# hidasib/GRU4Rec

Hardware: NVIDIA H100
Metric: mini-batches/sec (higher is better)
Workload: dtype f32

## Files before the change

### gru4rec_b200/csrc/g4r_fast.cuh

```cuda
#pragma once

constexpr int FK_THREADS = 512;
constexpr int FK_NW = FK_THREADS / 32;
constexpr int FK_G = 48;
constexpr int FK_CT = 32;
constexpr int FK_Q = FK_CT / FK_NW;
constexpr int FK_B = 32;
static_assert(FK_THREADS / 16 == FK_B, "statistics mapping: 16 threads per lane");
constexpr int FK_LDS = 132;


__device__ __forceinline__ void red_release_add(unsigned int* p, unsigned int v) {
  asm volatile("red.release.gpu.global.add.u32 [%0], %1;" :: "l"(p), "r"(v) : "memory");
}
__device__ __forceinline__ unsigned int atom_acqrel_add(unsigned int* p, unsigned int v) {
  unsigned int old;
  asm volatile("atom.acq_rel.gpu.global.add.u32 %0, [%1], %2;" : "=r"(old) : "l"(p), "r"(v) : "memory");
  return old;
}
__device__ __forceinline__ void wait_ge(const unsigned int* p, unsigned int target) {
  while (ld_acquire_u32(p) < target) { }
}
__device__ __forceinline__ uint32_t smem_u32(const void* p) { return (uint32_t)__cvta_generic_to_shared(p); }
__device__ __forceinline__ void mbar_init(uint64_t* bar, unsigned int count) {
  asm volatile("mbarrier.init.shared::cta.b64 [%0], %1;" :: "r"(smem_u32(bar)), "r"(count) : "memory");
}
__device__ __forceinline__ void mbar_expect_tx(uint64_t* bar, unsigned int bytes) {
  asm volatile("mbarrier.arrive.expect_tx.shared::cta.b64 _, [%0], %1;" :: "r"(smem_u32(bar)), "r"(bytes) : "memory");
}
__device__ __forceinline__ void mbar_wait(uint64_t* bar, unsigned int parity) {
  asm volatile(
      "{\n\t.reg .pred p;\n\t"
      "WAIT_LOOP:\n\t"
      "mbarrier.try_wait.parity.shared::cta.b64 p, [%0], %1;\n\t"
      "@p bra.uni WAIT_DONE;\n\t"
      "bra.uni WAIT_LOOP;\n\t"
      "WAIT_DONE:\n\t}\n" :: "r"(smem_u32(bar)), "r"(parity) : "memory");
}
__device__ __forceinline__ void tma_row(void* sdst, const void* gsrc, unsigned int bytes, uint64_t* bar) {
  asm volatile("cp.async.bulk.shared::cluster.global.mbarrier::complete_tx::bytes [%0], [%1], %2, [%3];"
               :: "r"(smem_u32(sdst)), "l"(gsrc), "r"(bytes), "r"(smem_u32(bar)) : "memory");
}

struct FastSmem {
  alignas(128) float sY[FK_B * FK_LDS];
  float sS[FK_CT * FK_LDS];
  float sAcc[FK_CT * FK_LDS];
  float sVel[FK_CT * FK_LDS];
  float sTW[FK_B * FK_LDS];
  float sD[FK_CT * FK_LDS];
  float sG[FK_CT * FK_B];
  float sO[FK_CT * FK_B];
  float sRS[FK_B * 8];
  float sPart[FK_NW * FK_B * 8];
// ... 597 lines not shown
    while (je < nj && sm.sIt[buf][je] == item) je++;
    if (lane < kw) {
      const float4 p0 = ld4(sm.sS + j * FK_LDS + lane * 4), z = make_float4(0.f, 0.f, 0.f, 0.f);
      RowChain<float4> u;
      u.begin(p0, p0, ada ? ld4(sm.sAcc + j * FK_LDS + lane * 4) : z, mom ? ld4(sm.sVel + j * FK_LDS + lane * 4) : z);
      for (int k = j; k < je; k++) u.add(md, ld4(sm.sD + k * FK_LDS + lane * 4), ada, mom);
      const size_t off = (size_t)item * ldL + lane * 4;
      st4(md.Wy + off, u.ps);
      if (ada) st4(md.Wy_acc + off, u.al);
      if (mom) st4(md.Wy_vel + off, u.vl);
    }
    if (lane == 0) {
      RowChain<float> u;
      u.begin(sm.sByP[j], sm.sByP[j], sm.sByA[j], sm.sByV[j]);
      for (int k = j; k < je; k++) u.add(md, sm.sDby[k], ada, mom);
      md.By[item] = u.ps;
      if (ada) md.By_acc[item] = u.al;
      if (mom) md.By_vel[item] = u.vl;
    }
  }
}
template <class SM>
__device__ __forceinline__ void fk_dby(SM& sm, int M, int nj) {
  const int lane = threadIdx.x & 31, warp = threadIdx.x >> 5;
  for (int jj = warp; jj < nj; jj += FK_NW) {
    float a = (lane < M) ? sm.sG[jj * FK_B + lane] : 0.f;
    a = warp_sum(a);
    if (lane == 0) sm.sDby[jj] = a;
  }
}
#include "g4r_fastc.cuh"

template <bool CL>
__global__ void __launch_bounds__(FK_THREADS, 1) k_fast_t(int slot, int n_steps, FastSync* fs, unsigned long long* tstamp) {
  using SM = typename std::conditional<CL, FastSmemC, FastSmemR>::type;
  extern __shared__ __align__(128) unsigned char fk_raw[];
  SM& sm = *reinterpret_cast<SM*>(fk_raw);
  const ModelDev& md = MD;
  const LayerDev& ly = md.layer[0];
  const int cta = blockIdx.x, ncta = gridDim.x;
  const int tid = threadIdx.x, lane = tid & 31, warp = tid >> 5;
  const int G = CL ? (int)cl_size() : md.ldL / 4;
  const bool gru = cta < G;
  const bool col = CL || !gru;
  const int chunk = CL ? cta : cta - G;
  const int ncol = CL ? ncta : ncta - G;
  const bool has_chunk = col && chunk < md.NCH;
  const bool pw = loss_pairwise(md.loss);
  const int ldL = md.ldL, B = md.B;
  const int kw = ldL / 4;
  uint64_t* bar = reinterpret_cast<uint64_t*>(&sm.mbar);
  unsigned int bar_epoch = 0, gepoch = 0, stats_target = 0;
  const int in_ctas = min(B, ncta - G);
#ifdef G4R_CF_FINE
#define FK_FTS(s_) ((tstamp && cta == 0 && (s_) < 500 && n_steps >= 1000) ? tstamp + (size_t)((s_) + 500) * 16 : nullptr)
#define FK_STAMP_OK(s_) ((s_) < 500)
#else
#define FK_FTS(s_) ((unsigned long long*)nullptr)
#define FK_STAMP_OK(s_) true
#endif
#define FK_STAMP(k) do { if (tstamp && cta == ((CL || ((k) >= 4 && (k) <= 8)) ? 0 : G) && tid == 0 && FK_STAMP_OK(s)) { unsigned long long t_; asm volatile("mov.u64 %0, %%globaltimer;" : "=l"(t_)); tstamp[(size_t)s * 16 + (k)] = t_; } } while (0)
  if (tid == 0) { mbar_init(bar, 1); asm volatile("fence.mbarrier_init.release.cluster;" ::: "memory"); }
  if (col) fk_load_idx(md, sm, 0, n_steps, chunk, 0);
  __syncthreads();
  if (col) fk_prefetch_rows(md, sm, 0, n_steps, 0, pw);
  ClusterCtx cc = {0, 1, 0, 0};
  if constexpr (CL) {
    if (gru) {
      cc = cf_init(md, sm);
      cf_load_resident(md, sm, cc);
      if (n_steps > 0) {
        fk_stage_lanes(md, sm, 0, md.wM[0]);
        cf_f1(md, sm, cc, 0, false, nullptr, 0u, nullptr);
        cf_f2(md, sm, cc, 0, nullptr);
        __syncthreads();
        if (tid == 0) red_release_add(&fs->h_ready, 1u);
      }
    }
  } else {
    if (gru) {
      fr_load_resident(md, sm, 4 * cta);
      if (n_steps > 0) {
        fk_stage_lanes(md, sm, 0, md.wM[0]);
        stage_rows4(sm.gH[0], FK_LDS, FK_B, kw, [&](int rr) -> const float* { const int sl = sm.gIdx[rr]; return sl >= 0 ? ly.H + (size_t)sl * ldL : nullptr; });
        fr_f1(md, sm, 0, 4 * cta, sm.gH[0], nullptr, 0u);
// ... 142 lines not shown
      const int b = chunk;
      const bool maxed = !(md.loss == G4R_LOSS_BPR || md.loss == G4R_LOSS_TOP1);
      float mc = -INFINITY, Z = 0.f, A = 0.f, Q = 0.f, D = 0.f, T = 0.f, has = 0.f, tt = 0.f;
      if (tid < md.NCH) {
        const float* st = md.stat + ((size_t)tid * md.B + b) * G4R_NSTAT;
        const float4 u = ld4(st), v = ld4(st + 4);
        mc = u.x; Z = u.y; A = u.z; Q = u.w; D = v.x; T = v.y; has = v.z;
        if (tid == 0) tt = v.w;
      }
      float mg = mc;
#pragma unroll
      for (int o = 1; o < 32; o <<= 1) mg = fmaxf(mg, __shfl_xor_sync(0xffffffffu, mg, o));
      if (lane == 0) sm.sPart[warp] = mg;
      __syncthreads();
      mg = sm.sPart[0];
      for (int w = 1; w < FK_NW; w++) mg = fmaxf(mg, sm.sPart[w]);
      if (loss_softmaxneg(md.loss)) mg = fmaxf(mg, 0.f);
      if (maxed) {
        const float sc = (mc == -INFINITY) ? 0.f : expf(mc - mg);
        Z *= sc; A *= sc; Q *= sc; D *= sc;
      }
#pragma unroll
      for (int o = 1; o < 32; o <<= 1) {
        Z += __shfl_xor_sync(0xffffffffu, Z, o); A += __shfl_xor_sync(0xffffffffu, A, o); Q += __shfl_xor_sync(0xffffffffu, Q, o);
        D += __shfl_xor_sync(0xffffffffu, D, o); T += __shfl_xor_sync(0xffffffffu, T, o); has += __shfl_xor_sync(0xffffffffu, has, o);
      }
      __syncthreads();
      if (lane == 0) { float* w = sm.sPart + 32 + warp * 8; w[0] = Z; w[1] = A; w[2] = Q; w[3] = D; w[4] = T; w[5] = has; w[6] = tt; }
      __syncthreads();
      if (tid == 0) {
        tt = sm.sPart[32 + 6];
        for (int w = 1; w < FK_NW; w++) { const float* q = sm.sPart + 32 + w * 8; Z += q[0]; A += q[1]; Q += q[2]; D += q[3]; T += q[4]; }
        const float m = mg;
        float* rs = md.RS + (size_t)b * G4R_NSTAT;
        float loss = 0.f, r0 = m, r1 = Z, r2 = 0.f, r3 = 0.f, r4 = 0.f, r5 = tt;
        if (md.loss == G4R_LOSS_XE) { const float pt = __fdiv_rn(expf(T - m), Z); loss = -logf(pt + G4R_EPS_LOG); r2 = pt; r5 = T; }
        else if (md.loss == G4R_LOSS_XE_LOGIT) { loss = logf(Z) - (T - m); r5 = T; }
        else if (md.loss == G4R_LOSS_BPR_MAX) { r2 = __fdiv_rn(A, Z); r3 = __fdiv_rn(Q, Z); r4 = __fdiv_rn(D, Z); loss = -logf(r2 + G4R_EPS_LOG) + md.bpreg * r3; }
        else if (md.loss == G4R_LOSS_TOP1_MAX) { r2 = __fdiv_rn(A, Z); r4 = __fdiv_rn(D, Z); loss = r2; }
        else if (md.loss == G4R_LOSS_BPR) { loss = A; r4 = D; }
        else { const float c = sigmoidf_(tt * tt); loss = (float)M * (__fdiv_rn(A, (float)N) - __fdiv_rn(c, (float)(M + md.S_cfg))); r4 = D; }
        st4(rs, make_float4(r0, r1, r2, r3));
        st4(rs + 4, make_float4(r4, r5, loss, 0.f));
        red_release_add(&fs->stats, 1u);
      }
    }
    stats_target += (unsigned int)M;
    if (tid == 0) wait_ge(&fs->stats, stats_target);
    __syncthreads();
    FK_STAMP(2);
    if (tid < M * 2) st4(sm.sRS + tid * 4, ld4(md.RS + tid * 4));
    __syncthreads();
    if (chunk == 0 && tid == 0) {
      float c = 0.f;
      for (int b = 0; b < M; b++) c += sm.sRS[b * 8 + 6];
      c = __fdiv_rn(c, (float)md.B);
      md.cost[s] = c;
      if (c != c) atomicExch(md.nanflag, 1);
    }
    FK_STAMP(11);
    for (int i = tid; i < FK_CT * FK_B; i += FK_THREADS) {
      const int jj = i / FK_B, b = i % FK_B;
      sm.sG[i] = (jj < nj && b < M) ? loss_grad_elem(md, sm.sRS + (size_t)b * 8, sm.sO[i], sm.sTc[buf][b] == cb + jj, M, N) : 0.f;
    }
    __syncthreads();
    fk_dby(sm, M, nj);
    FK_STAMP(12);
    float* part = md.part + (size_t)(has_chunk ? chunk : 0) * md.B * ldL;
    if constexpr (CL) {
      if (has_chunk) { fk_dsy(sm, M, nj, kw); fk_part(sm, part, M, nj, ldL); }
      __syncthreads();
      FK_STAMP(13);
      fk_update_rows(md, sm, buf, nj, kw);
      if (has_chunk && nj == 0) for (int i = tid; i < M * ldL; i += FK_THREADS) part[i] = 0.f;
      __syncthreads();
      FK_STAMP(14);
      bar_epoch += 1;
      if (tid == 0) { red_release_add(&fs->bar, 1u); wait_ge(&fs->bar, bar_epoch * (unsigned int)ncta); }
      __syncthreads();
      FK_STAMP(3);
      fk_b1<CL>(md, sm, s, cta, ncta);
      __syncthreads();
      if (tid == 0) red_release_add(&fs->b1_done, 1u);
      FK_STAMP(15);
      fk_prefetch_rows(md, sm, s + 1, n_steps, buf ^ 1, pw);
      FK_STAMP(4);
      if (gru) {
        if (s + 1 < n_steps) fk_stage_lanes(md, sm, s + 1, md.wM[s + 1]);
        cf_backward(md, sm, cc, fs, s, ncta, s + 1 < n_steps, (tstamp && cta == 0 && FK_STAMP_OK(s)) ? tstamp + (size_t)s * 16 : nullptr, FK_FTS(s));
        FK_STAMP(6);
        if (s + 1 < n_steps) {
          cf_f1(md, sm, cc, s + 1, true, &fs->in_done, (unsigned int)(s + 1) * (unsigned int)in_ctas, FK_FTS(s));
          FK_STAMP(7);
          cf_f2(md, sm, cc, s + 1, FK_FTS(s));
          __syncthreads();
          if (tid == 0) red_release_add(&fs->h_ready, 1u);
        } else {
          cl_wait();
        }
        FK_STAMP(8);
      }
      if (!gru && cta < G + in_ctas) {
        const unsigned int tgt = (unsigned int)(s + 1) * (unsigned int)G;
        if (in_ctas == B && ly.ld3 / 4 <= FK_THREADS) fk_sparse_in_one(md, sm, s, cta - G, &fs->grp, tgt);
        else {
          if (tid == 0) wait_ge(&fs->grp, tgt);
          __syncthreads();
          for (int b = cta - G; b < B; b += in_ctas) { fk_sparse_in(md, sm, s, b); __syncthreads(); }
        }
        __syncthreads();
        if (tid == 0) red_release_add(&fs->in_done, 1u);
      }
    } else {
      if (has_chunk) fk_part(sm, part, M, nj, ldL);
      if (has_chunk && nj == 0) for (int i = tid; i < M * ldL; i += FK_THREADS) part[i] = 0.f;
      __syncthreads();
      FK_STAMP(13);
      bar_epoch += 1;
      if (tid == 0) { red_release_add(&fs->bar, 1u); wait_ge(&fs->bar, bar_epoch * (unsigned int)ncol); }
      __syncthreads();
      FK_STAMP(3);
      fk_b1<CL>(md, sm, s, chunk, ncol);
      __syncthreads();
      if (tid == 0) red_release_add(&fs->b1_done, 1u);
      FK_STAMP(15);
      fk_dsy(sm, M, nj, kw);
      __syncthreads();
      if (chunk < in_ctas) {
        const unsigned int tgt = (unsigned int)(s + 1) * (unsigned int)G;
        if (in_ctas == B && ly.ld3 / 4 <= FK_THREADS) fk_sparse_in_one(md, sm, s, chunk, &fs->dvec_done, tgt);
        else {
          if (tid == 0) wait_ge(&fs->dvec_done, tgt);
          __syncthreads();
          for (int b = chunk; b < B; b += in_ctas) { fk_sparse_in(md, sm, s, b); __syncthreads(); }
        }
        __syncthreads();
        if (tid == 0) red_release_add(&fs->in_done, 1u);
      }
      fk_update_rows(md, sm, buf, nj, kw);
      __syncthreads();
      FK_STAMP(14);
      if (tid == 0) red_release_add(&fs->rows_done, 1u);
      if (s + 1 < n_steps) {
        if (tid == 0) wait_ge(&fs->rows_done, (unsigned int)(s + 1) * (unsigned int)ncol);
        __syncthreads();
        fk_prefetch_rows(md, sm, s + 1, n_steps, buf ^ 1, pw);
      }
    }
  }
  if constexpr (CL) { if (gru) cf_store_resident(md, sm, cc); }
  else { if (gru) fr_store_resident(md, sm, 4 * cta); }
#undef FK_STAMP
}
```

### gru4rec_b200/csrc/g4r_kernels.cuh

```cuda
#pragma once
#include <cuda_runtime.h>
#include <stdint.h>
#include "../../include/g4r.h"

#define G4R_EPS_LOG 1e-24f
#define G4R_NSTAT 8

struct ActSpec { int kind; float p1, p2; };
constexpr int MG_CAP = 256;
struct MgDev {
  int R, rank;
  int *gItem, *gPos, *gM, *gX;
  int *mEnt, *mItem, *mCbeg;
  int *mTot;
  int *xEnt, *xItem, *xTot;
  float *DSYall, *DBYall, *INall;
  float* gradFlat; size_t gradCount;
};

struct MgTensor { float *p, *acc, *vel; size_t goff; int count; };
struct TsBuf {
  unsigned char *A1, *A2, *A3, *A4, *A5, *A6, *A7, *A8;
  unsigned char *W1, *W2, *W3, *W4, *B3, *B4, *B5, *B8a, *B8b;
  float *P, *P1, *Pa, *Pb;
// ... 26 lines not shown

constexpr int MGS_MAXR = 8;
constexpr int MGS_FLAG_STRIDE = 32;
constexpr int MGS_GRU_CTAS = 48;
enum { MGF_ROWS = 0, MGF_APPLIED = MGS_MAXR, MGF_IN = 2 * MGS_MAXR, MGF_INAPPLIED = 3 * MGS_MAXR, MGF_DENSE = 4 * MGS_MAXR,
       MGF_COUNT = 4 * MGS_MAXR + MGS_MAXR * MGS_GRU_CTAS };
struct ShardDev {
  int R, rank, rows_local, ldW;
  int NA, DSL;
  float* W[MGS_MAXR];
  float* Wx[MGS_MAXR];
  float* inbox[MGS_MAXR];
  float* inboxIn[MGS_MAXR];
  float* denseIn[MGS_MAXR];
  float* mgInLL[MGS_MAXR];
  unsigned int* flags[MGS_MAXR];
  float *W_acc, *W_vel, *Wx_acc, *Wx_vel;
  float* mgIn;
  const int *aEnt, *aItem, *aCbeg;
  const int *xEnt, *xItem, *xTot;
  const int *gX, *gM;
  int* abort;
};
struct FastSync {
  unsigned int bar;      unsigned int p0[31];
  unsigned int stats;    unsigned int p1[31];
  unsigned int h_ready;  unsigned int p2[31];
  unsigned int b1_done;  unsigned int p3[31];
  unsigned int grp;      unsigned int p4[31];
  unsigned int in_done;  unsigned int p5[31];
  unsigned int dvec_done; unsigned int p6[31];
  unsigned int rows_done; unsigned int p7[31];
};
struct GridBar { unsigned int count; unsigned int gen; unsigned int pad[30]; };

struct LayerDev {
  int L, ldL, ld2, ld3;
  int in_dim, ld_in;
  float *Wx, *Wx_acc, *Wx_vel;
  float *Wh, *Wh_acc, *Wh_vel;
  float *Wrz, *Wrz_acc, *Wrz_vel;
  float *Bh, *Bh_acc, *Bh_vel;
  float *Wx_g, *Wh_g, *Wrz_g, *Bh_g;
  float *H;
  float *Hold, *r, *z, *ah, *ht, *y;
  float *dvec;
  float *dy;
  float *Hr;
  const float* in;
};

struct ModelDev {
  int n_items, n_layers, B, Bld, S, mode;
  int L, ldL;
  int in0_dim, ld_in0;
  int NP;
  int NCH;
  int loss; ActSpec fact, hact;
  float p_drop_h, p_drop_e, lr, mom, lmbd, bpreg, logq, alpha;
  int adapt; int nn_top1;
  float ap1, ap1c, ap2, ap2c;
  float grad_cap, smoothing;
  const float* gscale;
  float* gnorm2;
  float* stat2;
  int S_cfg;
// ... 1125 lines not shown
```

### gru4rec_b200/csrc/g4r_lib.cu

```cuda
#include <cuda_runtime.h>
#include <cub/device/device_radix_sort.cuh>
#include <algorithm>
#include <cmath>
#include <cstdio>
#include <cstring>
#include <map>
#include <mutex>
#include <string>
#include <vector>
#include "g4r_kernels.cuh"
#include "g4r_misc.cuh"

#define G4R_VERSION 102

static thread_local std::string g_create_error;
struct g4r_handle;
static void eval_release(g4r_handle* h);
static void sessions_release(g4r_handle* h);
static void mg_release(g4r_handle* h);
static void shard_release(g4r_handle* h);
static bool shard_eligible(const g4r_config& c, int n_sm);
static int shard_create(g4r_handle* h);
static bool tc_eligible(const g4r_config& c);
struct TensorInfo;
// ... 63 lines not shown
  std::string err;
  cudaStream_t stream = nullptr;
  cudaEvent_t ev0 = nullptr, ev1 = nullptr;
  char* ws = nullptr; size_t ws_bytes = 0; bool own_ws = false;
  size_t ws_off = 0;
  std::map<std::string, TensorInfo> tensors;
  int Bmax = 0, n_sm = 132;
  int CAP = 0;
  int *hX = nullptr, *hY = nullptr, *hSlot = nullptr, *hM = nullptr, *hSti = nullptr; uint8_t* hF = nullptr; uint32_t* hG = nullptr;
  float* hCost = nullptr;
  int *dX = nullptr, *dY = nullptr, *dSlot = nullptr, *dM = nullptr, *dSti = nullptr, *dXnext = nullptr; uint8_t *dF = nullptr, *dXflag = nullptr; uint32_t* dG = nullptr;
  int* dStepBase = nullptr;
  float *dP = nullptr, *dLogP0t = nullptr, *dLogP0s = nullptr, *dU = nullptr;
  int* dST = nullptr; int gen_len = 0; int64_t sample_ptr = 0; bool have_store = false; bool have_cdf = false;
  int32_t* dMrgState = nullptr; int n_streams = 0; bool mrg_init = false; int64_t mrg_rstate[6];
  float* He[G4R_MAX_LAYERS] = {};
  int* dRankCnt = nullptr; float* dTgt = nullptr;
  uint32_t global_step = 0;
  int win_steps = 0;
  int64_t launches = 0;
  int npow2 = 0;
  int slot = -1;
  cudaGraphExec_t graphU = nullptr, graph1 = nullptr; int graph_unroll = 16;
  bool use_graph = true;
  GridBar* dGridBar = nullptr; unsigned long long* dStamp = nullptr; int pk_blocks = 0; size_t pk_smem = 0;
  bool mg_alloc = false; MgDev mgdev; std::vector<MgTensor> mg_tensors;
  void* eval_ctx = nullptr;
  void* sessions = nullptr;
  uint64_t wy_version = 0;
  void* mg_host = nullptr;
  void* shard = nullptr;
  char* shard_ws = nullptr;
  size_t shard_ws_bytes = 0;
  FastSync* dFastSync = nullptr; bool fast_ok = false; bool fastc_ok = false; int fastc_grid = 0; int* hFlags = nullptr; int64_t fast_windows = 0, slow_windows = 0;
  bool prof = false; bool stamp_on = false;
  bool two_pass = false;
  bool phase_only = false;
  float* dGscale = nullptr;
  bool tc_ok = false; void* ts_buf = nullptr; unsigned long long* ts_dbg = nullptr; cudaStream_t side = nullptr, side2 = nullptr; cudaEvent_t ts_ev[12] = {};
  std::vector<cudaEvent_t> prof_ev; std::vector<int> prof_phase;
  BpttDev bw = {}; void* bptt_cub = nullptr; size_t bptt_cub_bytes = 0; int64_t bptt_windows = 0;
  FullDev fs = {}; int64_t full_steps = 0;
};

enum { PH_GATHER = 0, PH_F1, PH_F2, PH_SCORE, PH_STATS, PH_LOSSGRAD, PH_B1, PH_B2, PH_B3, PH_DENSE, PH_SPARSE_IN, PH_STATS2, PH_GRADCAP, PH_COUNT };
static const char* kPhaseNames[PH_COUNT] = {"gather_in", "gru_rz", "gru_h", "score", "stats", "lossgrad_update", "gru_bwd_elem", "gru_bwd_dHr", "gru_bwd_din", "dense_update", "sparse_in_update",
                                            "smoothing_stats", "grad_cap_norm_apply"};

#define LAUNCH_ON(strm, ph, ...) do { \
    cudaEvent_t e0_ = nullptr, e1_ = nullptr; \
    if (h->prof) { cudaEventCreate(&e0_); cudaEventCreate(&e1_); cudaEventRecord(e0_, (strm)); } \
    __VA_ARGS__; \
    h->launches++; \
    if (h->prof) { cudaEventRecord(e1_, (strm)); h->prof_ev.push_back(e0_); h->prof_ev.push_back(e1_); h->prof_phase.push_back(ph); } \
  } while (0)
#define LAUNCH(ph, ...) LAUNCH_ON(h->stream, ph, __VA_ARGS__)

#define CK(call) do { cudaError_t e_ = (call); if (e_ != cudaSuccess) { h->err = std::string(#call) + ": " + cudaGetErrorString(e_); return G4R_ERR_CUDA; } } while (0)
#define FAIL(code, msg) do { h->err = (msg); return (code); } while (0)

static inline int round4(int x) { return (x + 3) & ~3; }
static inline size_t align_up(size_t x, size_t a) { return (x + a - 1) / a * a; }

struct Carver {
  char* base; size_t off; bool dry;
  template <class T> T* take(size_t n) {
// ... 104 lines not shown
    ly.Hold = cv.take<float>((size_t)Bmax * ly.ldL); ly.r = cv.take<float>((size_t)Bmax * ly.ldL); ly.z = cv.take<float>((size_t)Bmax * ly.ldL);
    ly.ah = cv.take<float>((size_t)Bmax * ly.ldL); ly.ht = cv.take<float>((size_t)Bmax * ly.ldL); ly.y = cv.take<float>((size_t)Bmax * ly.ldL);
    ly.dvec = cv.take<float>((size_t)Bmax * ly.ld3); ly.dy = cv.take<float>((size_t)Bmax * ly.ldL); ly.Hr = cv.take<float>((size_t)Bmax * ly.ldL);
    reg("y" + si, ly.y, Bmax, L, ly.ldL); reg("dvec" + si, ly.dvec, Bmax, 3 * L, ly.ld3);
  }
  if (mode != 0) {
    md.Sx = cv.take<float>((size_t)Bmax * md.ld_in0); md.in0 = cv.take<float>((size_t)Bmax * md.ld_in0); md.dSx = cv.take<float>((size_t)Bmax * md.ld_in0);
    if (mode == 2) { md.snapAcc = cv.take<float>((size_t)Bmax * md.ld_in0); md.snapVel = cv.take<float>((size_t)Bmax * md.ld_in0); }
    reg("dSx", md.dSx, Bmax, md.in0_dim, md.ld_in0);
  }
  for (int i = 0; i < nl; i++) md.layer[i].in = (i == 0) ? md.in0 : md.layer[i - 1].y;
  md.O = cv.take<float>((size_t)NP * md.Bld);
  md.DSY = cv.take<float>((size_t)NP * ldL); md.DBY = cv.take<float>((size_t)NP);
  const FullDev fsh = full ? full_shape(c, n_sm) : FullDev{};
  md.part = cv.take<float>((size_t)std::max(NCH, fsh.ks) * B * ldL);
  md.stat = cv.take<float>((size_t)NCH * B * G4R_NSTAT);
  md.RS = cv.take<float>((size_t)Bmax * G4R_NSTAT);
  md.stat2 = md.smoothing > 0.f ? cv.take<float>((size_t)NCH * B * 2) : nullptr;
  float* gsc = c.grad_cap > 0.f ? cv.take<float>(8) : nullptr;
  md.gscale = gsc;
  md.cost = cv.take<float>((size_t)CAP);
  md.nanflag = cv.take<int>(4);
  reg("O", md.O, NP, Bmax, md.Bld); reg("DSY", md.DSY, NP, Llast, ldL);
  int* dX = cv.take<int>((size_t)CAP * B); int* dY = cv.take<int>((size_t)CAP * B); int* dSlot = cv.take<int>((size_t)CAP * B);
  int* dXnext = cv.take<int>((size_t)CAP * B);
  uint8_t* dF = cv.take<uint8_t>((size_t)CAP * B); uint8_t* dXflag = cv.take<uint8_t>((size_t)CAP * B);
  int* dM = cv.take<int>(CAP); int* dSti = cv.take<int>(CAP); uint32_t* dG = cv.take<uint32_t>(CAP);
  md.pItem = cv.take<int>((size_t)CAP * NP); md.pPos = cv.take<int>((size_t)CAP * NP);
  md.pTcol = cv.take<int>((size_t)CAP * B); md.pCbeg = cv.take<int>((size_t)CAP * (NCH + 1));
  md.pKey = shard ? cv.take<int>((size_t)CAP * NP) : nullptr;
  int* dStepBase = cv.take<int>(4);
  GridBar* dGridBar = cv.take<GridBar>(1);
  FastSync* dFastSync = cv.take<FastSync>(1);
  unsigned long long* dStamp = cv.take<unsigned long long>((size_t)CAP * 16);
  float* dP = cv.take<float>(c.n_items); float* dL0t = cv.take<float>(c.n_items); float* dL0s = cv.take<float>(c.n_items);
  int* dST = store ? cv.take<int>((size_t)gen_len * c.n_sample) : nullptr;
  float* dU = store ? cv.take<float>((size_t)gen_len * c.n_sample) : nullptr;
  int32_t* dMrg = cv.take<int32_t>((size_t)15360 * 6);
  MgDev mgd; memset(&mgd, 0, sizeof(mgd));
  std::vector<MgTensor> mgt;
  const bool twins = R > 1 || c.grad_cap > 0.f || c.bptt > 1;
  if (twins) {
    size_t cnt = 0;
    for (int i = 0; i < nl; i++) {
      const LayerDev& ly = md.layer[i];
      if (ly.in_dim > 0) cnt += (size_t)ly.in_dim * ly.ld3;
      cnt += (size_t)ly.L * ly.ldL + (size_t)ly.L * ly.ld2 + ly.ld3;
    }
    float* gf = cv.take<float>(cnt);
    size_t off = 0;
    for (int i = 0; i < nl; i++) {
      LayerDev& ly = md.layer[i];
      if (ly.in_dim > 0) { ly.Wx_g = gf ? gf + off : nullptr; mgt.push_back(MgTensor{ly.Wx, ly.Wx_acc, ly.Wx_vel, off, ly.in_dim * ly.ld3}); off += (size_t)ly.in_dim * ly.ld3; }
      ly.Wh_g = gf ? gf + off : nullptr; mgt.push_back(MgTensor{ly.Wh, ly.Wh_acc, ly.Wh_vel, off, ly.L * ly.ldL}); off += (size_t)ly.L * ly.ldL;
      ly.Wrz_g = gf ? gf + off : nullptr; mgt.push_back(MgTensor{ly.Wrz, ly.Wrz_acc, ly.Wrz_vel, off, ly.L * ly.ld2}); off += (size_t)ly.L * ly.ld2;
      ly.Bh_g = gf ? gf + off : nullptr; mgt.push_back(MgTensor{ly.Bh, ly.Bh_acc, ly.Bh_vel, off, ly.ld3}); off += ly.ld3;
    }
    mgd.R = R; mgd.rank = c.rank; mgd.gradFlat = gf; mgd.gradCount = cnt;
  }
  if (R > 1) {
    mgd.gItem = cv.take<int>((size_t)R * MG_CAP * NP); mgd.gPos = nullptr;
    mgd.gM = cv.take<int>((size_t)R * MG_CAP); mgd.gX = cv.take<int>((size_t)R * MG_CAP * B);
    mgd.mEnt = cv.take<int>((size_t)MG_CAP * R * NP); mgd.mItem = cv.take<int>((size_t)MG_CAP * R * NP);
    mgd.mCbeg = cv.take<int>((size_t)MG_CAP * (n_sm + 1)); mgd.mTot = cv.take<int>(MG_CAP);
    mgd.xEnt = cv.take<int>((size_t)MG_CAP * R * B); mgd.xItem = cv.take<int>((size_t)MG_CAP * R * B); mgd.xTot = cv.take<int>(MG_CAP);
    if (!shard) {
// ... 32 lines not shown
  BpttDev bw; memset(&bw, 0, sizeof(bw));
  if (c.bptt > 1) {
    const size_t TB = (size_t)c.bptt * B;
    for (int i = 0; i < nl; i++) {
      const LayerDev& ly = md.layer[i];
      bw.Hold[i] = cv.take<float>(TB * ly.ldL); bw.R[i] = cv.take<float>(TB * ly.ldL); bw.Z[i] = cv.take<float>(TB * ly.ldL);
      bw.Ah[i] = cv.take<float>(TB * ly.ldL); bw.Ht[i] = cv.take<float>(TB * ly.ldL);
      bw.In[i] = ly.in_dim > 0 ? cv.take<float>(TB * ly.ld_in) : nullptr;
      bw.Dvec[i] = cv.take<float>(TB * ly.ld3);
      bw.Carry[i] = cv.take<float>((size_t)B * ly.ldL); bw.Dyl[i] = cv.take<float>((size_t)B * ly.ldL);
      bw.Dh[i] = cv.take<float>((size_t)B * ly.ldL); bw.DHr[i] = cv.take<float>((size_t)B * ly.ldL);
    }
    bw.Dy = cv.take<float>(TB * ldL);
    bw.DSY = cv.take<float>((size_t)c.bptt * NP * ldL); bw.DBY = cv.take<float>((size_t)c.bptt * NP); bw.Item = cv.take<int>((size_t)c.bptt * NP);
    bw.DSx = mode != 0 ? cv.take<float>(TB * md.ld_in0) : nullptr;
    bw.M = cv.take<int>(c.bptt); bw.N = cv.take<int>(c.bptt); bw.X = cv.take<int>(TB); bw.Slot = cv.take<int>(TB);
    bw.F = cv.take<uint8_t>(TB); bw.G = cv.take<uint32_t>(c.bptt);
    bw.keys = cv.take<unsigned long long>((size_t)c.bptt * (B + NP)); bw.keys2 = cv.take<unsigned long long>((size_t)c.bptt * (B + NP));
  }
  FullDev fs = fsh;
  if (full) {
    fs.dO = cv.take<float>((size_t)c.n_items * md.Bld); fs.stat = cv.take<float>((size_t)fsh.tiles * B * 4);
    if (fsh.tc) {
      fs.Asplit = cv.take<unsigned char>((size_t)((B + FS_TC_M - 1) / FS_TC_M) * fsh.chunks * 2 * FS_TC_M * FS_TC_KC * 4);
      fs.Bsplit = cv.take<unsigned char>((size_t)((c.n_items + FS_TC_N - 1) / FS_TC_N) * fsh.chunks * 2 * FS_TC_N * FS_TC_KC * 4);
    }
  }
  int* dRank = cv.take<int>((size_t)Be * 4); float* dTgt = cv.take<float>((size_t)Be * 3);
  if (!cv.dry) {
    md.wX = dX; md.wY = dY; md.wSlot = dSlot; md.wM = dM; md.wSti = dSti; md.wXnext = dXnext; md.wF = dF; md.wXflag = dXflag; md.wG = dG;
    md.ST = dST; md.logP0t = dL0t; md.logP0s = dL0s;
    h->md = md; h->Bmax = Bmax; h->CAP = CAP; h->mg_alloc = R > 1; h->mgdev = mgd; h->mg_tensors = mgt; h->gen_len = store ? gen_len : 0;
    h->dX = dX; h->dY = dY; h->dSlot = dSlot; h->dM = dM; h->dSti = dSti; h->dXnext = dXnext; h->dF = dF; h->dXflag = dXflag; h->dG = dG;
    h->dGridBar = dGridBar; h->dStamp = dStamp; h->dFastSync = dFastSync;
    h->dStepBase = dStepBase; h->dP = dP; h->dLogP0t = dL0t; h->dLogP0s = dL0s; h->dST = dST; h->dU = dU; h->dMrgState = dMrg;
    h->dRankCnt = dRank; h->dTgt = dTgt;
    h->npow2 = next_pow2(B + S);
    h->shard_ws = shard_ws; h->shard_ws_bytes = shard_ws_bytes;
    h->tc_ok = tc;
    if (tc) { if (!h->ts_buf) h->ts_buf = new TsBuf(); *static_cast<TsBuf*>(h->ts_buf) = tsb; }
    h->bw = bw; h->fs = fs;
    h->dGscale = gsc; h->two_pass = c.grad_cap > 0.f; h->phase_only = c.grad_cap > 0.f || md.smoothing > 0.f || full;
  }
}

#define G4R_MAX_SLOTS 24
__constant__ ModelDev c_models[G4R_MAX_SLOTS];
static bool g_slot_used[G4R_MAX_SLOTS] = {};
static std::mutex g_slot_mutex;
static int slot_alloc() { std::lock_guard<std::mutex> lk(g_slot_mutex); for (int i = 0; i < G4R_MAX_SLOTS; i++) if (!g_slot_used[i]) { g_slot_used[i] = true; return i; } return -1; }
static void slot_free(int i) { std::lock_guard<std::mutex> lk(g_slot_mutex); if (i >= 0 && i < G4R_MAX_SLOTS) g_slot_used[i] = false; }
static cudaError_t slot_upload(int slot, const ModelDev& md, cudaStream_t st) {
  return cudaMemcpyToSymbolAsync(c_models, &md, sizeof(ModelDev), (size_t)slot * sizeof(ModelDev), cudaMemcpyHostToDevice, st);
}
#define MD (c_models[slot])
#define STEP_IDX (base ? (*base + off) : off)
__global__ void __launch_bounds__(256) k_gather_in(int slot, const int* base, int off, int train) { phase_gather_in(MD, STEP_IDX, train != 0, blockIdx.x, gridDim.x); }
__global__ void __launch_bounds__(GEMM_THREADS) k_f1(int slot, const int* base, int off, int li, float* Hsrc) {
  __shared__ float sA[GK * (GB + 1)], sB[GK * (GB + 1)];
  phase_f1(MD, li, STEP_IDX, Hsrc, blockIdx.x, sA, sB);
}
__global__ void __launch_bounds__(GEMM_THREADS) k_f2(int slot, const int* base, int off, int li, float* Hsrc, int train) {
  __shared__ float sA[GK * (GB + 1)], sB[GK * (GB + 1)];
  phase_f2(MD, li, STEP_IDX, Hsrc, train != 0, blockIdx.x, sA, sB);
}
__global__ void __launch_bounds__(SC_THREADS) k_score(int slot, const int* base, int off) {
  extern __shared__ __align__(16) float smem[];
// ... 859 lines not shown
  cudaGraph_t g = nullptr;
  CK(cudaStreamBeginCapture(h->stream, cudaStreamCaptureModeThreadLocal));
  const int64_t l0 = h->launches;
  for (int i = 0; i < unroll; i++) enqueue_train_step(h, h->dStepBase, i);
  k_advance<<<1, 32, 0, h->stream>>>(h->dStepBase, unroll);
  h->launches = l0;
  CK(cudaStreamEndCapture(h->stream, &g));
  CK(cudaGraphInstantiate(out, g, 0));
  cudaGraphDestroy(g);
  return G4R_OK;
}
static int64_t launches_per_step(const g4r_handle* h) {
  const ModelDev& md = h->md;
  if (h->tc_ok) return 25;
  if (h->cfg.full_softmax) return full_launches_per_step(h);
  int64_t n = (md.mode != 0 ? 1 : 0) + 4;
  for (int li = 0; li < md.n_layers; li++) n += 2 + 2 + (md.layer[li].in_dim > 0 ? 1 : 0) + 1;
  if (md.smoothing > 0.f) n += 2;
  if (h->two_pass) n += 3 + (int64_t)h->mg_tensors.size();
  return n;
}

static int run_window(g4r_handle* h, int64_t n) {
  bool fast = false, fastc = false;
  if ((h->cfg.step_mode == 3 && h->fastc_ok) || (h->cfg.step_mode == 2 && h->fast_ok)) {
    if (!h->prof) {
      CK(cudaMemcpyAsync(h->hFlags, h->md.nanflag, 4 * sizeof(int), cudaMemcpyDeviceToHost, h->stream));
      CK(cudaStreamSynchronize(h->stream));
      const bool fits = h->hFlags[2] <= FK_CT;
      fastc = fits && h->cfg.step_mode == 3;
      fast = fits && h->cfg.step_mode == 2;
    }
  }
  if (fastc) {
    int slot = h->slot, nst = (int)n; FastSync* fsp = h->dFastSync; unsigned long long* ts = h->stamp_on ? h->dStamp : nullptr;
    void* args[] = {&slot, &nst, &fsp, &ts};
    CK(cudaMemsetAsync(h->dFastSync, 0, sizeof(FastSync), h->stream));
    CK(fastc_launch(h->fastc_grid, h->stream, args));
    h->launches += 1; h->fast_windows++;
  } else if (fast) {
    int slot = h->slot, nst = (int)n; FastSync* fsp = h->dFastSync; unsigned long long* ts = h->stamp_on ? h->dStamp : nullptr;
    void* args[] = {&slot, &nst, &fsp, &ts};
    CK(cudaMemsetAsync(h->dFastSync, 0, sizeof(FastSync), h->stream));
    CK(cudaLaunchCooperativeKernel((void*)k_fast_t<false>, dim3(h->pk_blocks), dim3(FK_THREADS), args, sizeof(FastSmemR), h->stream));
    h->launches += 1; h->fast_windows++;
  } else if (h->cfg.step_mode >= 1 && !h->prof && h->pk_blocks > 0 && !h->phase_only && !h->tc_ok) {
    if (h->cfg.step_mode >= 2) h->slow_windows++;
    int slot = h->slot, nst = (int)n; GridBar* gb = h->dGridBar; unsigned long long* ts = h->stamp_on ? h->dStamp : nullptr;
    void* args[] = {&slot, &nst, &gb, &ts};
    CK(cudaMemsetAsync(h->dGridBar, 0, sizeof(GridBar), h->stream));
    CK(cudaLaunchCooperativeKernel((void*)k_persistent, dim3(h->pk_blocks), dim3(PK_THREADS), args, h->pk_smem, h->stream));
    h->launches += 1;
  } else if (h->prof || !h->use_graph) {
    for (int64_t i = 0; i < n; i++) enqueue_train_step(h, nullptr, (int)i);
  } else {
    if (!h->graphU) { int rc = build_graph(h, h->graph_unroll, &h->graphU); if (rc) return rc; rc = build_graph(h, 1, &h->graph1); if (rc) return rc; }
    CK(cudaMemsetAsync(h->dStepBase, 0, sizeof(int), h->stream));
    int64_t i = 0;
    for (; i + h->graph_unroll <= n; i += h->graph_unroll) CK(cudaGraphLaunch(h->graphU, h->stream));
    for (; i < n; i++) CK(cudaGraphLaunch(h->graph1, h->stream));
    h->launches += n * launches_per_step(h) + (n / h->graph_unroll) + (n % h->graph_unroll);
  }
  CK(cudaGetLastError());
  if (h->gen_len > 0) h->sample_ptr += n;
  h->global_step += (uint32_t)n;
  if (h->cfg.full_softmax) h->full_steps += n;
  return G4R_OK;
}

#include "g4r_multi.cuh"
#include "g4r_shard.cuh"
#include "g4r_bptt.cuh"
static bool mg_is_ready(g4r_handle* h) { return h->mg_host && static_cast<MgHost*>(h->mg_host)->ready; }

extern "C" int g4r_upload_steps(g4r_handle* h, const g4r_schedule* s, int64_t first, int64_t n) {
  if (!h || !s) return G4R_ERR_INVALID;
  if (h->shard && n > MG_CAP) FAIL(G4R_ERR_INVALID, "row-sharded handle: at most MG_CAP steps per uploaded window");
// ... 275 lines not shown
```

Before: 32190.

## Replace stats counter barrier with tagged per-word row statistics polling

Row statistics used to be written to a float buffer and followed by a release-add on a global counter, and one thread then spun until all rows had arrived before the statistics were copied into shared memory. Now each statistic is written as a 64-bit word carrying a step tag, and each consumer thread polls its own word until the tag matches, loading it straight into shared memory. This removes one global atomic round trip and one block barrier per step. In the non-cluster path the dby reduction is also moved to later, after the b1_done signal, so it drops off the critical path; the host keeps a running tag base and clears the buffer when the tag would wrap.

New measurement: 32890 (median of 6 runs). About the same (+2.2%).

```diff
diff --git a/gru4rec_b200/csrc/g4r_fast.cuh b/gru4rec_b200/csrc/g4r_fast.cuh
--- a/gru4rec_b200/csrc/g4r_fast.cuh
+++ b/gru4rec_b200/csrc/g4r_fast.cuh
@@ -7,6 +7,7 @@
 constexpr int FK_Q = FK_CT / FK_NW;
 constexpr int FK_B = 32;
 static_assert(FK_THREADS / 16 == FK_B, "statistics mapping: 16 threads per lane");
+static_assert(FK_B * 7 <= FK_THREADS && FK_B * 8 <= FAST_RS_WORDS, "tagged row statistics: one word per thread");
 constexpr int FK_LDS = 132;
 
 
@@ -20,6 +21,15 @@
 }
 __device__ __forceinline__ void wait_ge(const unsigned int* p, unsigned int target) {
   while (ld_acquire_u32(p) < target) { }
+}
+__device__ __forceinline__ void st_tag(unsigned long long* p, float v, unsigned int tag) {
+  const unsigned long long w = ((unsigned long long)tag << 32) | __float_as_uint(v);
+  asm volatile("st.relaxed.gpu.global.b64 [%0], %1;" :: "l"(p), "l"(w) : "memory");
+}
+__device__ __forceinline__ float poll_tag(const unsigned long long* p, unsigned int tag) {
+  unsigned long long w;
+  do { asm volatile("ld.relaxed.gpu.global.b64 %0, [%1];" : "=l"(w) : "l"(p) : "memory"); } while ((unsigned int)(w >> 32) != tag);
+  return __uint_as_float((unsigned int)w);
 }
 __device__ __forceinline__ uint32_t smem_u32(const void* p) { return (uint32_t)__cvta_generic_to_shared(p); }
 __device__ __forceinline__ void mbar_init(uint64_t* bar, unsigned int count) {
@@ -683,7 +693,7 @@
 #include "g4r_fastc.cuh"
 
 template <bool CL>
-__global__ void __launch_bounds__(FK_THREADS, 1) k_fast_t(int slot, int n_steps, FastSync* fs, unsigned long long* tstamp) {
+__global__ void __launch_bounds__(FK_THREADS, 1) k_fast_t(int slot, int n_steps, FastSync* fs, unsigned long long* tstamp, unsigned long long* tRS, unsigned int tbase) {
   using SM = typename std::conditional<CL, FastSmemC, FastSmemR>::type;
   extern __shared__ __align__(128) unsigned char fk_raw[];
   SM& sm = *reinterpret_cast<SM*>(fk_raw);
@@ -701,7 +711,7 @@
   const int ldL = md.ldL, B = md.B;
   const int kw = ldL / 4;
   uint64_t* bar = reinterpret_cast<uint64_t*>(&sm.mbar);
-  unsigned int bar_epoch = 0, gepoch = 0, stats_target = 0;
+  unsigned int bar_epoch = 0, gepoch = 0;
   const int in_ctas = min(B, ncta - G);
 #ifdef G4R_CF_FINE
 #define FK_FTS(s_) ((tstamp && cta == 0 && (s_) < 500 && n_steps >= 1000) ? tstamp + (size_t)((s_) + 500) * 16 : nullptr)
@@ -910,7 +920,6 @@
         tt = sm.sPart[32 + 6];
         for (int w = 1; w < FK_NW; w++) { const float* q = sm.sPart + 32 + w * 8; Z += q[0]; A += q[1]; Q += q[2]; D += q[3]; T += q[4]; }
         const float m = mg;
-        float* rs = md.RS + (size_t)b * G4R_NSTAT;
         float loss = 0.f, r0 = m, r1 = Z, r2 = 0.f, r3 = 0.f, r4 = 0.f, r5 = tt;
         if (md.loss == G4R_LOSS_XE) { const float pt = __fdiv_rn(expf(T - m), Z); loss = -logf(pt + G4R_EPS_LOG); r2 = pt; r5 = T; }
         else if (md.loss == G4R_LOSS_XE_LOGIT) { loss = logf(Z) - (T - m); r5 = T; }
@@ -918,17 +927,15 @@
         else if (md.loss == G4R_LOSS_TOP1_MAX) { r2 = __fdiv_rn(A, Z); r4 = __fdiv_rn(D, Z); loss = r2; }
         else if (md.loss == G4R_LOSS_BPR) { loss = A; r4 = D; }
         else { const float c = sigmoidf_(tt * tt); loss = (float)M * (__fdiv_rn(A, (float)N) - __fdiv_rn(c, (float)(M + md.S_cfg))); r4 = D; }
-        st4(rs, make_float4(r0, r1, r2, r3));
-        st4(rs + 4, make_float4(r4, r5, loss, 0.f));
-        red_release_add(&fs->stats, 1u);
-      }
-    }
-    stats_target += (unsigned int)M;
-    if (tid == 0) wait_ge(&fs->stats, stats_target);
+        unsigned long long* rs = tRS + (size_t)b * 8;
+        const unsigned int tg = tbase + (unsigned int)s + 1u;
+        st_tag(rs + 0, r0, tg); st_tag(rs + 1, r1, tg); st_tag(rs + 2, r2, tg); st_tag(rs + 3, r3, tg);
+        st_tag(rs + 4, r4, tg); st_tag(rs + 5, r5, tg); st_tag(rs + 6, loss, tg);
+      }
+    }
+    if (tid < M * 7) sm.sRS[(tid / 7) * 8 + tid % 7] = poll_tag(tRS + (tid / 7) * 8 + tid % 7, tbase + (unsigned int)s + 1u);
     __syncthreads();
     FK_STAMP(2);
-    if (tid < M * 2) st4(sm.sRS + tid * 4, ld4(md.RS + tid * 4));
-    __syncthreads();
     if (chunk == 0 && tid == 0) {
       float c = 0.f;
       for (int b = 0; b < M; b++) c += sm.sRS[b * 8 + 6];
@@ -942,7 +949,7 @@
       sm.sG[i] = (jj < nj && b < M) ? loss_grad_elem(md, sm.sRS + (size_t)b * 8, sm.sO[i], sm.sTc[buf][b] == cb + jj, M, N) : 0.f;
     }
     __syncthreads();
-    fk_dby(sm, M, nj);
+    if constexpr (CL) fk_dby(sm, M, nj);
     FK_STAMP(12);
     float* part = md.part + (size_t)(has_chunk ? chunk : 0) * md.B * ldL;
     if constexpr (CL) {
@@ -1002,6 +1009,7 @@
       __syncthreads();
       if (tid == 0) red_release_add(&fs->b1_done, 1u);
       FK_STAMP(15);
+      fk_dby(sm, M, nj);
       fk_dsy(sm, M, nj, kw);
       __syncthreads();
       if (chunk < in_ctas) {
diff --git a/gru4rec_b200/csrc/g4r_kernels.cuh b/gru4rec_b200/csrc/g4r_kernels.cuh
--- a/gru4rec_b200/csrc/g4r_kernels.cuh
+++ b/gru4rec_b200/csrc/g4r_kernels.cuh
@@ -82,6 +82,7 @@
   unsigned int dvec_done; unsigned int p6[31];
   unsigned int rows_done; unsigned int p7[31];
 };
+constexpr int FAST_RS_WORDS = 32 * 8;
 struct GridBar { unsigned int count; unsigned int gen; unsigned int pad[30]; };
 
 struct LayerDev {
diff --git a/gru4rec_b200/csrc/g4r_lib.cu b/gru4rec_b200/csrc/g4r_lib.cu
--- a/gru4rec_b200/csrc/g4r_lib.cu
+++ b/gru4rec_b200/csrc/g4r_lib.cu
@@ -119,6 +119,7 @@
   void* shard = nullptr;
   char* shard_ws = nullptr;
   size_t shard_ws_bytes = 0;
+  unsigned long long* dFastRS = nullptr; uint32_t fast_tag = 0;
   FastSync* dFastSync = nullptr; bool fast_ok = false; bool fastc_ok = false; int fastc_grid = 0; int* hFlags = nullptr; int64_t fast_windows = 0, slow_windows = 0;
   bool prof = false; bool stamp_on = false;
   bool two_pass = false;
@@ -289,6 +290,7 @@
   int* dStepBase = cv.take<int>(4);
   GridBar* dGridBar = cv.take<GridBar>(1);
   FastSync* dFastSync = cv.take<FastSync>(1);
+  unsigned long long* dFastRS = cv.take<unsigned long long>(FAST_RS_WORDS);
   unsigned long long* dStamp = cv.take<unsigned long long>((size_t)CAP * 16);
   float* dP = cv.take<float>(c.n_items); float* dL0t = cv.take<float>(c.n_items); float* dL0s = cv.take<float>(c.n_items);
   int* dST = store ? cv.take<int>((size_t)gen_len * c.n_sample) : nullptr;
@@ -387,7 +389,7 @@
     md.ST = dST; md.logP0t = dL0t; md.logP0s = dL0s;
     h->md = md; h->Bmax = Bmax; h->CAP = CAP; h->mg_alloc = R > 1; h->mgdev = mgd; h->mg_tensors = mgt; h->gen_len = store ? gen_len : 0;
     h->dX = dX; h->dY = dY; h->dSlot = dSlot; h->dM = dM; h->dSti = dSti; h->dXnext = dXnext; h->dF = dF; h->dXflag = dXflag; h->dG = dG;
-    h->dGridBar = dGridBar; h->dStamp = dStamp; h->dFastSync = dFastSync;
+    h->dGridBar = dGridBar; h->dStamp = dStamp; h->dFastSync = dFastSync; h->dFastRS = dFastRS;
     h->dStepBase = dStepBase; h->dP = dP; h->dLogP0t = dL0t; h->dLogP0s = dL0s; h->dST = dST; h->dU = dU; h->dMrgState = dMrg;
     h->dRankCnt = dRank; h->dTgt = dTgt;
     h->npow2 = next_pow2(B + S);
@@ -1313,17 +1315,18 @@
       fast = fits && h->cfg.step_mode == 2;
     }
   }
-  if (fastc) {
+  if (fastc || fast) {
+    if ((uint64_t)h->fast_tag + (uint64_t)n > 0xFFFFFFFFull) {
+      CK(cudaMemsetAsync(h->dFastRS, 0, FAST_RS_WORDS * sizeof(unsigned long long), h->stream));
+      h->fast_tag = 0;
+    }
     int slot = h->slot, nst = (int)n; FastSync* fsp = h->dFastSync; unsigned long long* ts = h->stamp_on ? h->dStamp : nullptr;
-    void* args[] = {&slot, &nst, &fsp, &ts};
+    unsigned long long* trs = h->dFastRS; unsigned int tbase = h->fast_tag;
+    void* args[] = {&slot, &nst, &fsp, &ts, &trs, &tbase};
     CK(cudaMemsetAsync(h->dFastSync, 0, sizeof(FastSync), h->stream));
-    CK(fastc_launch(h->fastc_grid, h->stream, args));
-    h->launches += 1; h->fast_windows++;
-  } else if (fast) {
-    int slot = h->slot, nst = (int)n; FastSync* fsp = h->dFastSync; unsigned long long* ts = h->stamp_on ? h->dStamp : nullptr;
-    void* args[] = {&slot, &nst, &fsp, &ts};
-    CK(cudaMemsetAsync(h->dFastSync, 0, sizeof(FastSync), h->stream));
-    CK(cudaLaunchCooperativeKernel((void*)k_fast_t<false>, dim3(h->pk_blocks), dim3(FK_THREADS), args, sizeof(FastSmemR), h->stream));
+    if (fastc) CK(fastc_launch(h->fastc_grid, h->stream, args));
+    else CK(cudaLaunchCooperativeKernel((void*)k_fast_t<false>, dim3(h->pk_blocks), dim3(FK_THREADS), args, sizeof(FastSmemR), h->stream));
+    h->fast_tag += (uint32_t)n;
     h->launches += 1; h->fast_windows++;
   } else if (h->cfg.step_mode >= 1 && !h->prof && h->pk_blocks > 0 && !h->phase_only && !h->tc_ok) {
     if (h->cfg.step_mode >= 2) h->slow_windows++;
```
